# urgent-challenge/urgent2026_challenge_track1

Measured on AMD Instinct MI355X. Metric: utterances/sec (4 s @ 48 kHz) train step, higher is better.
Workload: dtype bf16

## Files before the change

include/urse.h:

```cpp
#ifndef URSE_H_
#define URSE_H_
#include <stdint.h>

#ifdef __cplusplus
extern "C" {
#endif

#define URSE_OK 0
#define URSE_ERR_INVALID_ARG (-1)
#define URSE_ERR_LAUNCH (-2)
#define URSE_ERR_UNSUPPORTED (-3)
#define URSE_ERR_RUNTIME (-4)

#define URSE_F32 0
#define URSE_BF16 1
#define URSE_F16 2
#define URSE_BF16_ACT_F16 3

#define URSE_WIN_RECT 0
#define URSE_WIN_HANN 1

int urse_version(void);
const char* urse_last_error(void);

#define URSE_KV_NT_BRES 0
#define URSE_KV_NT_RING 1
#define URSE_KV_NT_RING_WIDE 2
#define URSE_KV_NT_128 3
#define URSE_KV_NT_GROUPED_RING 4
#define URSE_KV_NT_GROUPED_128 5
#define URSE_KV_TN_RING 6
#define URSE_KV_TN_RING_T 7
#define URSE_KV_TN_DUAL 8
#define URSE_KV_TN_128 9
#define URSE_KV_TN_GROUPED 10
#define URSE_KV_LSTM_FWD_STREAM 11
#define URSE_KV_LSTM_FWD_WIDE 12
#define URSE_KV_LSTM_FWD_CLUSTER 13
#define URSE_KV_LSTM_FWD_CLUSTER2 14
#define URSE_KV_LSTM_BWD_STREAM16 15
#define URSE_KV_LSTM_BWD_STREAM32 16
#define URSE_KV_LSTM_BWD_CLUSTER 17
#define URSE_KV_LSTM_BWD_SPLIT 18
#define URSE_KV_STFT960 19
#define URSE_KV_STFT_GENERIC 20
#define URSE_KV_ISTFT_GENERIC 21
#define URSE_KV_ISTFT960 22
#define URSE_KV_LSTM_FWD_RW 23
#define URSE_KV_TN_ACT_F16 24
#define URSE_KV_LSTM_FWD_RWX 25
#define URSE_KV_LSTM_BWD_NSPLIT 26
#define URSE_KV_LSTM_FWD_CLUSTERX 27
#define URSE_KV_COUNT 32
int urse_launch_count(int variant);
int urse_launch_counts_reset(void);

int urse_stft_fwd(const float* wav, const int32_t* lens, float* spec, int B, int L, int n_fft, int hop,
                  int window, void* stream);
int urse_istft_fwd(const float* spec, float* wav, int B, int T, int n_fft, int hop, int L_out, int window,
                   void* stream);
int urse_istft_bwd(const float* grad_wav, float* grad_spec, int B, int T, int n_fft, int hop, int L_out,
                   int window, void* stream);

int urse_gemm_nt(const void* A, int64_t lda, const void* B, int64_t ldb, void* C, int64_t ldc, const float* bias,
                 const float* resid, int64_t ldr, int64_t M, int64_t N, int64_t K, int in_dtype, int out_dtype,
                 int act, void* stream);
int urse_gemm_nt_gnstats(const void* A, int64_t lda, const void* B, int64_t ldb, float* C, int64_t ldc, const float* bias,
                         const float* resid, int64_t ldr, int64_t M, int64_t N, int64_t K, int in_dtype, int act,
                         double* stats, int64_t rows_per_group, void* stream);
int urse_gemm_nt_gnbwd(const void* A, int64_t lda, const void* B, int64_t ldb, float* C, int64_t M, int64_t N, int64_t K, int in_dtype,
                       const float* x, const double* stats, const float* gamma, double* sums, float* dgamma, float* dbeta, float* part,
                       int slots, int64_t rows_per_group, float eps, void* stream);
int urse_gemm_nt_grouped(const void* descs, int groups, int max_blocks, int in_dtype, int out_dtype, int act,
                         void* stream);
int urse_gemm_nt_grouped_h(const void* descs, const int64_t* host_descs, int groups, int in_dtype, int out_dtype,
                           int act, void* stream);
int urse_gemm_tn(const void* A, int64_t lda, const void* B, int64_t ldb, float* C, int64_t ldc, float* colsum,
                 int64_t R, int64_t Mo, int64_t No, int64_t shift, int64_t inner, int64_t period,
                 int64_t invalid_step, int64_t perm_h, int dtype, int target_workgroups, void* stream);
int urse_gemm_tn_act_f16_supported(int64_t R, int64_t Mo, int64_t No, int64_t No2, int with_colsum, int64_t inner, int64_t period);
int urse_gemm_tn_dual(const void* A, int64_t lda, const void* B, int64_t ldb, float* C, int64_t ldc, float* colsum,
                      const void* B2, int64_t ldb2, float* C2, int64_t ldc2, int64_t R, int64_t Mo, int64_t No, int64_t No2,
                      int64_t shift, int64_t inner, int64_t period, int64_t invalid_step, int64_t perm_h, int dtype,
                      int target_workgroups, void* stream);
int urse_gemm_tn_grouped(const void* descs, int groups, int max_blocks, int dtype, void* stream);

int urse_groupnorm_fwd(const float* x, const float* gamma, const float* beta, const float* add, void* y, double* stats,
                       int B, int T, int Kg, int W, int N, int Np, int gstride, float eps, int out_dtype, void* y_bf16, void* stream);
int urse_groupnorm_stats(const float* x, double* stats, int B, int T, int Kg, int W, int N, void* stream);
int urse_groupnorm_apply(const float* x, const float* gamma, const float* beta, const float* add, void* y, const double* stats,
                         int B, int T, int Kg, int W, int N, int Np, int gstride, float eps, int out_dtype, void* y_bf16, void* stream);
int urse_groupnorm_bwd(const float* x, const float* dy, const double* stats, const float* gamma, const float* dres,
                       float* dx, float* dgamma, float* dbeta, double* sums, int B, int T, int Kg, int W, int N,
                       int gstride, float eps, void* dx_packed, int ldp, void* stream);
int urse_groupnorm_bwd_apply(const float* x, const float* dy, const double* stats, const double* sums, const float* gamma,
                             const float* dres, float* dx, int B, int T, int Kg, int W, int N, int gstride, float eps, void* dx_packed,
                             int ldp, void* stream);
int urse_pack2d(const void* in, int64_t ldi, int in_dtype, void* out, int64_t ldo, int out_dtype, int rows, int cols,
                int out_rows, int out_cols, int transpose, void* stream);

int urse_pack_segments(const float* in, void* out, const void* segs, int nseg, int blocks_per_seg, int transpose,
                       int out_dtype, void* stream);

int urse_lstm_pack(const float* wih, const float* whh, const float* bih, const float* bhh, void* wih_p, void* wihT_p,
                   float* bias, void* whh_frag, void* whhT_frag, int N, int Np, int H, int Hp, int dtype,
                   void* stream);

int urse_lstm_bidir_fwd(void* gx, int64_t ldg, const void* whh, void* hout, int64_t ldh, float* c, int H, int Hp,
                        int n_seq, int seq_len, int64_t inner, int64_t outer, int64_t stride, int save, int dtype,
                        int rows16, void* hout_bf16, void* stream);
int urse_lstm_pack_quads(const float* whh, void* out, int H, int Hp, int dtype, void* stream);
int urse_lstm_cluster_plan(int H, int Hp, int n_seq, int reserved_cus, int64_t* plan);
int urse_lstm_cluster_fwd(void* gx, int64_t ldg, const void* whhq, void* hout, int64_t ldh, float* c, void* hx,
                          void* counters, void* err_flag, int H, int Hp, int n_seq, int seq_len, int64_t inner,
                          int64_t outer, int64_t stride, int save, int reserved_cus, int xcd_aware, int dtype, void* hout_bf16,
                          void* stream);
int urse_lstm_clusterx_supported(int N, int Np, int H, int Hp);
int urse_lstm_clusterx_plan(int H, int Hp, int n_seq, int reserved_cus, int64_t* plan);
int urse_lstm_clusterx_hx_elems(int H, int Hp, int n_seq, int reserved_cus, int64_t* elems);
int urse_lstm_pack_quads_x(const float* wih, void* out, int N, int Np, int H, int dtype, void* stream);
int urse_lstm_clusterx_fwd(const void* xn, int64_t ldx, const void* wihq, const float* bias, const void* whhq, void* gates, int64_t ldg, void* hout,
                           int64_t ldh, float* c, void* hx, void* counters, void* err_flag, int N, int Np, int H, int Hp, int n_seq, int seq_len,
                           int64_t inner, int64_t outer, int64_t stride, int save, int reserved_cus, int xcd_aware, int dtype, void* hout_bf16,
                           void* stream);
int urse_lstm_cluster2_plan(int H, int Hp, int n_seq, int reserved_cus, int64_t* plan);
int urse_lstm_cluster2_fwd(void* gx, int64_t ldg, const void* whhq, void* hout, int64_t ldh, float* c, void* hx, void* err_flag,
                           int H, int Hp, int n_seq, int seq_len, int64_t inner, int64_t outer, int64_t stride, int save,
                           int reserved_cus, int dtype, void* stream);
int urse_lstm_pack_bwd_quads(const float* whh, void* out, int H, int C, void* stream);
int urse_lstm_cluster_bwd(const void* dh, int64_t ldd, void* gates, int64_t ldg, const float* c, const void* whhTq,
                          void* dgx, void* counters, void* err_flag, int H, int Hp, int n_seq, int seq_len, int64_t inner,
                          int64_t outer, int64_t stride, int reserved_cus, void* stream);
int urse_lstm_wide_supported(int H, int Hp);
int urse_lstm_pack_blocks(const float* whh, void* out, int H, int Hp, void* stream);
int urse_lstm_wide_fwd(void* gx, int64_t ldg, const void* whhb, void* hout, int64_t ldh, float* c, int H, int Hp,
// ... 146 lines not shown
```

urgent2026_challenge_track1_amd/csrc/gemm.hip:

```cpp
#include <stdlib.h>

#include <type_traits>
#include "urse_common.h"

namespace urse {

typedef __bf16 bf16x8_t __attribute__((ext_vector_type(8)));
typedef short short8_t __attribute__((ext_vector_type(8)));
typedef short short4_t __attribute__((ext_vector_type(4)));
typedef float f32x4_t __attribute__((ext_vector_type(4)));

struct GemmDesc {
  const char* A;
  const char* B;
  char* C;
  const float* bias;
  const float* resid;
  long lda, ldb, ldc;
  long M, N, K;
  long ldr;
};

constexpr int BM = 128, BN = 128;
constexpr int SLAB = 64;
// ... 1470 lines not shown
          }
        } else {
          const TO* sv = reinterpret_cast<const TO*>(src);
          for (int e = 0; e < EPC && col + e < d.N; ++e) {
            float f = to_f32<TO>(sv[e]);
            if (OS == 4 && d.resid && ACT != 2) f += d.resid[row * d.ldr + col + e];
            if (gst) {
              if (row < gbound) { gsa += f; gqa += f * f; } else { gsb += f; gqb += f * f; }
            }
            C[row * d.ldc + col + e] = from_f32<TO>(f);
            if constexpr (C2K) {
              if (C2) C2[row * d.ldr + col + e] = f32_to_bf16(f);
            }
          }
        }
      }
      ch += DCH;
      if (ch >= CPR) { ch -= CPR; ++lrow; }
    }
  }
  if constexpr (GNB) {
    __syncthreads();
    constexpr int SLOTS = NTHR / CPR;
    double* red = reinterpret_cast<double*>(lds);
    float4* pg = reinterpret_cast<float4*>(lds + 1024);
    float4* pb = pg + SLOTS * CPR;
    const double r0 = wave_sum_d((double)gsa), r1 = wave_sum_d((double)gqa), r2 = wave_sum_d((double)gsb), r3 = wave_sum_d((double)gqb);
    if (lane == 0) { red[w * 4] = r0; red[w * 4 + 1] = r1; red[w * 4 + 2] = r2; red[w * 4 + 3] = r3; }
    if (tid < SLOTS * CPR) {
      pg[tid] = make_float4(gnb_dg[0], gnb_dg[1], gnb_dg[2], gnb_dg[3]);
      pb[tid] = make_float4(gnb_db[0], gnb_db[1], gnb_db[2], gnb_db[3]);
    }
    __syncthreads();
    if (tid < 4) {
      double t = 0.0;
      for (int i = 0; i < NWV; ++i) t += red[i * 4 + tid];
      const long g = gnb_g0 + (tid >> 1);
      if ((tid < 2 || gnb_bound < m0 + BMX) && g * xt->rpg < d.M) atomicAdd(xt->gnb_sums + g * 2 + (tid & 1), t);
    }
    if (tid >= 64 && tid < 64 + CPR) {
      const int chf = tid - 64;
      const long col = n0 + chf * EPC;
      if (col < d.N) {
        float4 sg = make_float4(0.f, 0.f, 0.f, 0.f), sb = sg;
        for (int i = 0; i < SLOTS; ++i) {
          const float4 a = pg[i * CPR + chf], bq = pb[i * CPR + chf];
          sg.x += a.x; sg.y += a.y; sg.z += a.z; sg.w += a.w;
          sb.x += bq.x; sb.y += bq.y; sb.z += bq.z; sb.w += bq.w;
        }
        float* part = xt->gnb_part + (long)(blockIdx.x % xt->gnb_slots) * 2 * d.N;
        const float vg[4] = {sg.x, sg.y, sg.z, sg.w}, vb[4] = {sb.x, sb.y, sb.z, sb.w};
        for (int q = 0; q < 4 && col + q < d.N; ++q) {
          atomicAdd(part + col + q, vg[q]);
          atomicAdd(part + d.N + col + q, vb[q]);
        }
      }
    }
    return;
  }
  if (gst) {
    __syncthreads();
    double* red = reinterpret_cast<double*>(lds);
    const double r0 = wave_sum_d((double)gsa), r1 = wave_sum_d((double)gqa), r2 = wave_sum_d((double)gsb), r3 = wave_sum_d((double)gqb);
    if (lane == 0) { red[w * 4] = r0; red[w * 4 + 1] = r1; red[w * 4 + 2] = r2; red[w * 4 + 3] = r3; }
    __syncthreads();
    if (tid < 4) {
      double t = 0.0;
      for (int i = 0; i < NWV; ++i) t += red[i * 4 + tid];
      const long g = gidx + (tid >> 1);
      if (tid < 2 || gbound < m0 + BMX) {
        if (g * rpg < d.M) atomicAdd(gstats + g * 2 + (tid & 1), t);
      }
    }
  }
}

template <typename TO, int NTW, int ACT, int BMX, int WNC = 2, typename TI = bf16_t>
__global__ void __launch_bounds__(BMX / 64 * WNC * 64) gemm_nt_dma_kernel(GemmDesc d, NtExtra x) {
  gemm_nt_dma_body<TO, NTW, ACT, BMX, WNC, 0, TI>(d, x.gstats, x.rpg);
}

__global__ void __launch_bounds__(512) gemm_nt_dma_gnb_kernel(GemmDesc d, NtExtra x) {
  gemm_nt_dma_body<float, 7, 0, 256, 2, 1>(d, nullptr, 0, &x);
}

__global__ void gnb_fold_kernel(const float* __restrict__ part, int slots, int N, float* __restrict__ dgamma, float* __restrict__ dbeta) {
  const int c = blockIdx.x * blockDim.x + threadIdx.x;
  if (c >= N) return;
  float a = 0.f, b = 0.f;
  for (int s = 0; s < slots; ++s) { a += part[(long)s * 2 * N + c]; b += part[(long)s * 2 * N + N + c]; }
  dgamma[c] += a;
  dbeta[c] += b;
}

template <typename TO, int ACT, typename TI = bf16_t>
__global__ void __launch_bounds__(512) gemm_nt_dma_grouped_kernel(const GemmDesc* __restrict__ descs) {
  const GemmDesc d = descs[blockIdx.y];
  gemm_nt_dma_body<TO, 7, ACT, 256, 2, 0, TI>(d);
}

template <int ACT, typename TI = bf16_t>
__global__ void __launch_bounds__(512) gemm_nt_bres_kernel(GemmDesc d, int wg_per_slice) {
  constexpr int BMX = 256, NTW = 7, BNX = 224, NST = 3, STAGE = BMX * 64, KSTEPS = 7, BRES = KSTEPS * 14 * 1024;
  __shared__ __attribute__((aligned(1024))) char lds[BRES + NST * STAGE];
  char* ring = lds + BRES;
  const int tm = (int)((d.M + BMX - 1) / BMX);
  const int tile_n = blockIdx.x / wg_per_slice, part = blockIdx.x - tile_n * wg_per_slice;
  const long n0 = (long)tile_n * BNX;
  const int tid = threadIdx.x, lane = tid & 63;
  const int w = __builtin_amdgcn_readfirstlane(tid >> 6), wm = w >> 1, wn = w & 1;
  const int nk = (int)(d.K / 32);
  const char* zsrc = reinterpret_cast<const char*>(g_tn_zero_page) + lane * 16;
  const int srow = lane >> 2, schunk = (lane & 3) ^ ((lane >> 3) & 3);
  const int lc = lane & 15, lr = lane >> 4;
  const int foff = lc * 64 + ((lr ^ ((lc >> 1) & 3)) << 4);
  for (int blk = w; blk < nk * 14; blk += 8) {
    const int kt = blk / 14, b = blk - kt * 14;
    const long row = n0 + b * 16 + srow;
    glds16(row < d.N ? d.B + (row * d.ldb) * 2 + schunk * 16 + (long)kt * 64 : zsrc, lds + blk * 1024);
  }
  f32x4_t bv[NTW];
#pragma unroll
  for (int j = 0; j < NTW; ++j) {
    const long col = n0 + (wn * NTW + j) * 16 + lr * 4;
#pragma unroll
    for (int r = 0; r < 4; ++r) bv[j][r] = (d.bias && col + r < d.N) ? d.bias[col + r] : 0.f;
  }
  bf16_t* C = reinterpret_cast<bf16_t*>(d.C);
  auto tile_src = [&](int mt, const char* (&pa)[2], bool (&aok)[2]) __attribute__((always_inline)) {
#pragma unroll
    for (int j = 0; j < 2; ++j) {
      const long row = (long)mt * BMX + 16 * (2 * w + j) + srow;
      aok[j] = mt < tm && row < d.M;
      pa[j] = d.A + (row * d.lda) * 2 + schunk * 16;
    }
  };
  auto issue = [&](const char* (&pa)[2], bool (&aok)[2], int kt, int slot) __attribute__((always_inline)) {
#pragma unroll
    for (int j = 0; j < 2; ++j)
      glds16((kt < nk && aok[j]) ? pa[j] + (long)kt * 64 : zsrc, ring + slot * STAGE + (2 * w + j) * 1024);
  };
  const char* pa[2];
  bool aok[2];
  tile_src(part, pa, aok);
  issue(pa, aok, 0, 2);
  for (int mt = part; mt < tm; mt += wg_per_slice) {
    const long m0 = (long)mt * BMX;
    issue(pa, aok, 1, 0);
    f32x4_t acc[4][NTW];
#pragma unroll
    for (int i = 0; i < 4; ++i)
#pragma unroll
      for (int j = 0; j < NTW; ++j) acc[i][j] = f32x4_t{0.f, 0.f, 0.f, 0.f};
    int slot = 2;
    for (int kt = 0; kt < nk; ++kt) {
      asm volatile("s_waitcnt vmcnt(2)" ::: "memory");
      __builtin_amdgcn_s_barrier();
      int nslot = slot + 2;
      if (nslot >= NST) nslot -= NST;
      issue(pa, aok, kt + 2, nslot);
      const char* As = ring + slot * STAGE + wm * 4096 + foff;
      const char* Bs = lds + kt * (14 * 1024) + wn * NTW * 1024 + foff;
      short8_t a[4], b[NTW];
#pragma unroll
      for (int i = 0; i < 4; ++i) a[i] = *reinterpret_cast<const short8_t*>(As + i * 1024);
#pragma unroll
// ... 227 lines not shown
  else { set_error("gemm_nt: bad dtype %d/%d", in_dtype, out_dtype); return URSE_ERR_INVALID_ARG; }
  URSE_CHECK_LAUNCH("urse_gemm_nt");
  return URSE_OK;
}

static long g_nt_bres_min_n = getenv("URSE_NT_BRES_MIN_N") ? atol(getenv("URSE_NT_BRES_MIN_N")) : 448;
static int g_nt_bres_wgs = 256;
static int g_nt_wide_default = 1;
static long g_nt_wide_maxk = 256;

static int gemm_nt_impl(const void* A, int64_t lda, const void* B, int64_t ldb, void* C, int64_t ldc,
                        const float* bias, const float* resid, int64_t ldr, int64_t M, int64_t N, int64_t K,
                        int in_dtype, int out_dtype, int act, void* stream, double* gstats, long rpg, int* fused) {
  NtExtra xtra{};
  GemmDesc d;
  d.A = (const char*)A; d.B = (const char*)B; d.C = (char*)C; d.bias = bias; d.resid = resid;
  d.lda = lda; d.ldb = ldb; d.ldc = ldc; d.M = M; d.N = N; d.K = K; d.ldr = ldr;
  const bool in16 = in_dtype == URSE_BF16 || in_dtype == URSE_F16;
  const bool f16 = in_dtype == URSE_F16;
  URSE_CHECK_ARG(in16 || in_dtype == URSE_F32, "urse_gemm_nt: bad operand dtype %d", in_dtype);
  URSE_CHECK_ARG(out_dtype == URSE_F32 || (out_dtype == URSE_BF16 && !f16) || (out_dtype == URSE_F16 && f16),
                 "urse_gemm_nt: output dtype %d with operand dtype %d (16-bit outputs take the operands' format)", out_dtype, in_dtype);
  const bool out16 = out_dtype != URSE_F32;
  int rc = check_desc_host(d, in16 ? 2 : 4, "urse_gemm_nt");
  if (rc) return rc;
  URSE_CHECK_ARG(!resid || act == 2 || out_dtype == URSE_F32 || (in_dtype == URSE_F16 && out_dtype == URSE_F16 && act == 1),
                 "urse_gemm_nt: residual epilogue writes f32 (f16 operands with act 1: the aux slot is the bf16 copy of the output)");
  URSE_CHECK_ARG(act != 2 || resid, "urse_gemm_nt: act 2 (tanh backward) needs the aux operand");
  static const bool no_dma = getenv("URSE_NT_NO_DMA") != nullptr;
  const char* bres_env = getenv("URSE_NT_BRES");
  const int bres_mode = bres_env ? atoi(bres_env) : 1;
#ifdef URSE_EXPERIMENTS
  const long wreg_min_n = getenv("URSE_NT_WREG_MIN_N") ? atol(getenv("URSE_NT_WREG_MIN_N")) : 0;
  if (wreg_min_n > 0 && in_dtype == URSE_BF16 && out_dtype == URSE_BF16 && !no_dma && M >= 8192 && N >= wreg_min_n && K == 32 * WR_KS &&
      !resid && act != 2 && (ldc * 2) % 16 == 0 && ((uintptr_t)C % 16) == 0 && M * lda * 2 < 0xFFFFF000L && M * ldc * 2 < 0xFFFFF000L) {
    const int tn = (int)((N + WR_BNX - 1) / WR_BNX);
    int parts = 252 / tn;
    if (parts < 1) parts = 1;
    long rpp = (M + parts - 1) / parts;
    rpp = (rpp + WR_ROWS - 1) / WR_ROWS * WR_ROWS;
    dim3 grid((unsigned)(tn * parts));
    hipStream_t st = (hipStream_t)stream;
    note_launch(URSE_KV_NT_BRES);
    if (act == 0) hipLaunchKernelGGL(gemm_nt_wreg_kernel<0>, grid, dim3(448), 0, st, d, parts, rpp);
    else hipLaunchKernelGGL(gemm_nt_wreg_kernel<1>, grid, dim3(448), 0, st, d, parts, rpp);
    URSE_CHECK_LAUNCH("urse_gemm_nt");
    return URSE_OK;
  }
#endif
  if (bres_mode && in16 && out16 && !no_dma && M >= 8192 && N >= g_nt_bres_min_n && K % 32 == 0 &&
      K >= 96 && K <= 224 && !resid && act != 2 && (ldc * 2) % 16 == 0 && ((uintptr_t)C % 16) == 0) {
    const int tn = (int)((N + 223) / 224);
    int per = g_nt_bres_wgs / tn;
    if (per < 1) per = 1;
    dim3 grid((unsigned)(tn * per));
    hipStream_t st = (hipStream_t)stream;
    note_launch(URSE_KV_NT_BRES);
    if (f16) {
      if (act == 0) hipLaunchKernelGGL((gemm_nt_bres_kernel<0, f16_t>), grid, dim3(512), 0, st, d, per);
      else hipLaunchKernelGGL((gemm_nt_bres_kernel<1, f16_t>), grid, dim3(512), 0, st, d, per);
    } else if (act == 0) hipLaunchKernelGGL(gemm_nt_bres_kernel<0>, grid, dim3(512), 0, st, d, per);
    else hipLaunchKernelGGL(gemm_nt_bres_kernel<1>, grid, dim3(512), 0, st, d, per);
    URSE_CHECK_LAUNCH("urse_gemm_nt");
    return URSE_OK;
  }
  if (in16 && !no_dma && M >= 2048 && N >= 160 && K % 32 == 0 && K >= 96 && !(f16 && act == 2)) {
    const long pad7 = (N + 223) / 224 * 224, pad8 = (N + 255) / 256 * 256;
    int ntw = pad7 <= pad8 ? 7 : 8;
    if (const char* e = getenv("URSE_NT_NTW")) ntw = atoi(e) == 8 ? 8 : 7;
    int bmx = 256;
    if (const char* e = getenv("URSE_NT_BMX")) bmx = atoi(e) == 128 ? 128 : 256;
    int wide = g_nt_wide_default && K <= g_nt_wide_maxk && N >= 1792 && out_dtype == URSE_BF16 && (N + 447) / 448 * 448 <= pad7 + 64;
    if (const char* e = getenv("URSE_NT_WIDE")) wide = atoi(e) != 0 && N >= 448;
    if (f16) { wide = 0; bmx = 256; }
    const long tl = wide ? ((M + 127) / 128) * ((N + 447) / 448) : ((M + bmx - 1) / bmx) * ((N + 32L * ntw - 1) / (32L * ntw));
    URSE_CHECK_ARG(tl < (1L << 31), "urse_gemm_nt: too many tiles");
    dim3 grid((unsigned)tl);
    hipStream_t st = (hipStream_t)stream;
    if (gstats && out_dtype == URSE_F32 && act != 2 && !wide && rpg >= bmx) {
      xtra.gstats = gstats;
      xtra.rpg = rpg;
      if (fused) *fused = 1;
    }
#define URSE_NT_DMA(TO_, NTW_, ACT_, BMX_) \
  hipLaunchKernelGGL((gemm_nt_dma_kernel<TO_, NTW_, ACT_, BMX_>), grid, dim3(BMX_ * 2), 0, st, d, xtra)
#define URSE_NT_DMA_W(TO_, ACT_) \
  hipLaunchKernelGGL((gemm_nt_dma_kernel<TO_, 7, ACT_, 128, 4>), grid, dim3(512), 0, st, d, xtra)
#define URSE_NT_DMA_B(TO_, NTW_, ACT_) do { if (wide) URSE_NT_DMA_W(TO_, ACT_); else if (bmx == 128) URSE_NT_DMA(TO_, NTW_, ACT_, 128); else URSE_NT_DMA(TO_, NTW_, ACT_, 256); } while (0)
#define URSE_NT_DMA_ACT(TO_, NTW_) \
  do { if (act == 0) URSE_NT_DMA_B(TO_, NTW_, 0); else if (act == 1) URSE_NT_DMA_B(TO_, NTW_, 1); else URSE_NT_DMA_B(TO_, NTW_, 2); } while (0)
    note_launch(wide ? URSE_KV_NT_RING_WIDE : URSE_KV_NT_RING);
    if (f16) {
#define URSE_NT_DMA_H(TO_, NTW_, ACT_) hipLaunchKernelGGL((gemm_nt_dma_kernel<TO_, NTW_, ACT_, 256, 2, f16_t>), grid, dim3(512), 0, st, d, xtra)
#define URSE_NT_DMA_H_ACT(TO_, NTW_) do { if (act == 0) URSE_NT_DMA_H(TO_, NTW_, 0); else URSE_NT_DMA_H(TO_, NTW_, 1); } while (0)
      if (out_dtype == URSE_F16) { if (ntw == 7) URSE_NT_DMA_H_ACT(f16_t, 7); else URSE_NT_DMA_H_ACT(f16_t, 8); }
      else { if (ntw == 7) URSE_NT_DMA_H_ACT(float, 7); else URSE_NT_DMA_H_ACT(float, 8); }
    } else if (out_dtype == URSE_BF16) {
      if (ntw == 7) URSE_NT_DMA_ACT(bf16_t, 7); else URSE_NT_DMA_ACT(bf16_t, 8);
    } else {
      if (ntw == 7) URSE_NT_DMA_ACT(float, 7); else URSE_NT_DMA_ACT(float, 8);
    }
    URSE_CHECK_LAUNCH("urse_gemm_nt");
    return URSE_OK;
  }
  const long blocks = ((M + BM - 1) / BM) * ((N + BN - 1) / BN);
  URSE_CHECK_ARG(blocks < (1L << 31), "urse_gemm_nt: too many tiles");
  note_launch(URSE_KV_NT_128);
  return dispatch_nt(nullptr, d, 1, (int)blocks, in_dtype, out_dtype, act, (hipStream_t)stream);
}

extern "C" int urse_gemm_nt(const void* A, int64_t lda, const void* B, int64_t ldb, void* C, int64_t ldc,
                            const float* bias, const float* resid, int64_t ldr, int64_t M, int64_t N, int64_t K,
                            int in_dtype, int out_dtype, int act, void* stream) {
  return gemm_nt_impl(A, lda, B, ldb, C, ldc, bias, resid, ldr, M, N, K, in_dtype, out_dtype, act, stream, nullptr, 0, nullptr);
}

extern "C" int urse_gemm_nt_gnstats(const void* A, int64_t lda, const void* B, int64_t ldb, float* C, int64_t ldc,
                                    const float* bias, const float* resid, int64_t ldr, int64_t M, int64_t N, int64_t K,
                                    int in_dtype, int act, double* stats, int64_t rows_per_group, void* stream) {
  URSE_CHECK_ARG(stats && rows_per_group > 0 && M % rows_per_group == 0 && ldc == N && N % 4 == 0,
                 "urse_gemm_nt_gnstats: needs whole groups of rows, a dense output and N %% 4 == 0");
  const int groups = (int)(M / rows_per_group);
  (void)hipMemsetAsync(stats, 0, sizeof(double) * 2 * groups, (hipStream_t)stream);
  int fused = 0;
  int rc = gemm_nt_impl(A, lda, B, ldb, C, ldc, bias, resid, ldr, M, N, K, in_dtype, URSE_F32, act, stream, stats, rows_per_group,
                        &fused);
  if (rc || fused) return rc;
  return urse_groupnorm_stats(C, stats, groups, (int)rows_per_group, 1, (int)N, (int)N, stream);
}

extern "C" int urse_gemm_nt_gnbwd(const void* A, int64_t lda, const void* B, int64_t ldb, float* C, int64_t M, int64_t N, int64_t K,
                                  int in_dtype, const float* x, const double* stats, const float* gamma, double* sums, float* dgamma,
                                  float* dbeta, float* part, int slots, int64_t rows_per_group, float eps, void* stream) {
  URSE_CHECK_ARG(A && B && C && x && stats && gamma && sums && dgamma && dbeta && part && slots > 0 && rows_per_group > 0,
                 "urse_gemm_nt_gnbwd: bad argument");
  static const bool no_dma = getenv("URSE_NT_NO_DMA") != nullptr;
  if (no_dma || in_dtype != URSE_BF16 || M < 2048 || N < 160 || N > 224 || N % 4 || K % 32 || K < 96 || rows_per_group < 256 ||
      M % rows_per_group || ((uintptr_t)C % 16) || ((uintptr_t)x % 16)) {
    set_error("urse_gemm_nt_gnbwd: shape M%ld N%ld K%ld not served by the fused kernel", (long)M, (long)N, (long)K);
    return URSE_ERR_UNSUPPORTED;
  }
  GemmDesc d;
  d.A = (const char*)A; d.B = (const char*)B; d.C = (char*)C; d.bias = nullptr; d.resid = nullptr;
  d.lda = lda; d.ldb = ldb; d.ldc = N; d.M = M; d.N = N; d.K = K; d.ldr = 0;
  int rc = check_desc_host(d, 2, "urse_gemm_nt_gnbwd");
  if (rc) return rc;
  hipStream_t st = (hipStream_t)stream;
  const size_t sums_bytes = sizeof(double) * 2 * (size_t)(M / rows_per_group), part_bytes = sizeof(float) * 2 * (size_t)N * slots;
  if (reinterpret_cast<char*>(part) == reinterpret_cast<char*>(sums) + sums_bytes) {
    (void)hipMemsetAsync(sums, 0, sums_bytes + part_bytes, st);
  } else {
    (void)hipMemsetAsync(sums, 0, sums_bytes, st);
    (void)hipMemsetAsync(part, 0, part_bytes, st);
  }
  NtExtra xt{};
  xt.rpg = rows_per_group; xt.gnb_x = x; xt.gnb_stats = stats; xt.gnb_gamma = gamma; xt.gnb_sums = sums; xt.gnb_part = part;
  xt.gnb_slots = slots; xt.gnb_eps = eps;
  const long tl = (M + 255) / 256;
  URSE_CHECK_ARG(tl < (1L << 31), "urse_gemm_nt_gnbwd: too many tiles");
  note_launch(URSE_KV_NT_RING);
  hipLaunchKernelGGL(gemm_nt_dma_gnb_kernel, dim3((unsigned)tl), dim3(512), 0, st, d, xt);
  hipLaunchKernelGGL(gnb_fold_kernel, dim3((unsigned)((N + 255) / 256)), dim3(256), 0, st, part, slots, (int)N, dgamma, dbeta);
  URSE_CHECK_LAUNCH("urse_gemm_nt_gnbwd");
  return URSE_OK;
}

// ... 251 lines not shown
```

urgent2026_challenge_track1_amd/ops.py:

```python
import os

import torch

from . import _lib
from ._lib import call, require_cuda, stream_ptr

WIN_RECT, WIN_HANN = 0, 1
F32, BF16, F16 = 0, 1, 2
BF16_ACT_F16 = 3
HALF_TYPES = (torch.bfloat16, torch.float16)


def bwd_dtype(dtype):
    return torch.bfloat16 if dtype == torch.float16 else dtype

_timing = None


def enable_timing(names):
    global _timing
    _timing = {n: [] for n in names}


def disable_timing():
    global _timing
    t, _timing = _timing, None
    return t


def timed_call(tname, name, *args):
    if _timing is not None and tname in _timing:
        a, b = torch.cuda.Event(enable_timing=True), torch.cuda.Event(enable_timing=True)
        a.record()
        call(name, *args)
        b.record()
        _timing[tname].append((a, b))
    else:
        call(name, *args)


KERNEL_VARIANTS = ("nt_bres", "nt_ring", "nt_ring_wide", "nt_128", "nt_grouped_ring", "nt_grouped_128", "tn_ring", "tn_ring_t",
                   "tn_dual", "tn_128", "tn_grouped", "lstm_fwd_stream", "lstm_fwd_wide", "lstm_fwd_cluster",
                   "lstm_fwd_cluster2", "lstm_bwd_stream16", "lstm_bwd_stream32", "lstm_bwd_cluster", "lstm_bwd_split",
                   "stft960", "stft_generic", "istft_generic", "istft960", "lstm_fwd_rw", "tn_act_f16", "lstm_fwd_rwx", "lstm_bwd_nsplit",
                   "lstm_fwd_clusterx", "_unused28")


_PAGEABLE_UPLOADS = os.environ.get("URSE_PAGEABLE_UPLOADS", "0") == "1"


def upload(host_tensor, device, cached=False):
    if torch.device(device).type != "cuda":
        return host_tensor
    if _PAGEABLE_UPLOADS:
        return host_tensor.to(device)
    out = host_tensor.contiguous().pin_memory().to(device, non_blocking=True)
    if cached:
        ev = torch.cuda.Event()
        ev.record(torch.cuda.current_stream(device))
        ev.synchronize()
    return out


def launch_counts(reset=False):
    lib = _lib.load()
    out = {n: lib.urse_launch_count(i) for i, n in enumerate(KERNEL_VARIANTS)}
    if reset:
        lib.urse_launch_counts_reset()
    return out


def _f32c(t):
    return t.contiguous().float() if (t.dtype != torch.float32 or not t.is_contiguous()) else t


def stft_forward(wav, n_fft, hop, window=WIN_HANN, lens=None):
    require_cuda(wav)
    wav = _f32c(wav)
    B, L = wav.shape
    T, Fb = L // hop + 1, n_fft // 2 + 1
    spec = torch.empty(B, T, Fb, 2, device=wav.device, dtype=torch.float32)
    if lens is not None:
        if lens.device.type == "cpu":
            lens = upload(lens.to(torch.int32), wav.device)
        else:
            lens = lens.to(device=wav.device, dtype=torch.int32).contiguous()
    timed_call("stft_fwd", "stft_fwd", wav, lens, spec, B, L, n_fft, hop, window, stream_ptr())
    return torch.view_as_complex(spec)


class _ISTFT(torch.autograd.Function):
    @staticmethod
    def forward(ctx, spec_ri, n_fft, hop, length, window):
        B, T, Fb, _ = spec_ri.shape
        wav = torch.empty(B, length, device=spec_ri.device, dtype=torch.float32)
        call("istft_fwd", spec_ri, wav, B, T, n_fft, hop, length, window, stream_ptr())
        ctx.cfg = (B, T, Fb, n_fft, hop, length, window)
        return wav

    @staticmethod
    def backward(ctx, g):
        B, T, Fb, n_fft, hop, length, window = ctx.cfg
        g = _f32c(g)
        gs = torch.empty(B, T, Fb, 2, device=g.device, dtype=torch.float32)
        call("istft_bwd", g, gs, B, T, n_fft, hop, length, window, stream_ptr())
        return gs, None, None, None, None


def istft_forward(spec, n_fft, hop, length, window=WIN_HANN):
    if spec.is_complex():
        spec = torch.view_as_real(spec)
    require_cuda(spec)
    return _ISTFT.apply(_f32c(spec), n_fft, hop, int(length), window)


def _dt(t):
    if t.dtype == torch.bfloat16:
        return BF16
    if t.dtype == torch.float32:
        return F32
    if t.dtype == torch.float16:
        return F16
    raise TypeError("URSE GEMM operands are bf16, f16 or f32, got %s" % t.dtype)


def dtype_code(dtype):
    return {torch.float32: F32, torch.bfloat16: BF16, torch.float16: F16}[dtype]

# ... 882 lines not shown
```

Before: 256.1.

## Add persistent streaming NT GEMM kernel for narrow fp32 outputs with residual

Adds a persistent NT GEMM kernel that launches one workgroup per CU and loops over M tiles. The next tile's first K slabs are prefetched into the LDS ring while the current tile's epilogue runs, and the epilogue is staged through LDS so bias, residual and group-norm stats are applied in coalesced row sweeps with nontemporal stores. It is on by default for fp32-output, no-activation, N<=224 GEMMs that have a residual and enough tiles. The aim is to remove per-tile launch and drain overhead and to hide epilogue memory traffic, at the cost of extra barriers and fewer workgroups per CU.

```diff
diff --git a/include/urse.h b/include/urse.h
--- a/include/urse.h
+++ b/include/urse.h
@@ -51,6 +51,7 @@
 #define URSE_KV_LSTM_FWD_RWX 25
 #define URSE_KV_LSTM_BWD_NSPLIT 26
 #define URSE_KV_LSTM_FWD_CLUSTERX 27
+#define URSE_KV_NT_STREAM 28
 #define URSE_KV_COUNT 32
 int urse_launch_count(int variant);
 int urse_launch_counts_reset(void);
diff --git a/urgent2026_challenge_track1_amd/csrc/gemm.hip b/urgent2026_challenge_track1_amd/csrc/gemm.hip
--- a/urgent2026_challenge_track1_amd/csrc/gemm.hip
+++ b/urgent2026_challenge_track1_amd/csrc/gemm.hip
@@ -1576,6 +1576,187 @@
 
 __global__ void __launch_bounds__(512) gemm_nt_dma_gnb_kernel(GemmDesc d, NtExtra x) {
   gemm_nt_dma_body<float, 7, 0, 256, 2, 1>(d, nullptr, 0, &x);
+}
+
+template <int NTW, typename TI>
+__global__ void __launch_bounds__(512) gemm_nt_stream_kernel(GemmDesc d, NtExtra x) {
+  constexpr int BMX = 256, BNX = 32 * NTW, NWV = 8, NTHR = 512, NST = 4, STAGE = (BMX + 256) * 64, BOFF = BMX * 64;
+  constexpr int AI = 2, BI = 2;
+  constexpr int CP = BNX * 4 + 16, RPP = 32, STG = RPP * CP, CPR = BNX / 4;
+  constexpr int SW = (RPP * CPR + NTHR - 1) / NTHR;
+  static_assert(NST * STAGE + STG + BNX * 4 <= 160 * 1024, "ring + staging buffer + bias row exceed the LDS");
+  static_assert(BMX % (2 * RPP) == 0 && 2 * RPP == 64, "a wave's 64 rows are two passes");
+  __shared__ __attribute__((aligned(1024))) char lds[NST * STAGE + STG + BNX * 4];
+  char* const stg = lds + NST * STAGE;
+  const long tm = (d.M + BMX - 1) / BMX;
+  const long t0 = (long)blockIdx.x * tm / gridDim.x, t1 = ((long)blockIdx.x + 1) * tm / gridDim.x;
+  if (t0 >= t1) return;
+  const int tid = threadIdx.x, lane = tid & 63;
+  const int w = __builtin_amdgcn_readfirstlane(tid >> 6), wm = w >> 1, wn = w & 1;
+  const int nk = (int)(d.K / 32);
+  const char* zsrc = reinterpret_cast<const char*>(g_tn_zero_page) + lane * 16;
+  const int srow = lane >> 2, schunk = (lane & 3) ^ ((lane >> 3) & 3);
+  const int lc = lane & 15, lr = lane >> 4;
+  const int foff = lc * 64 + ((lr ^ ((lc >> 1) & 3)) << 4);
+
+  const char* pa[AI];
+  const char* pb[BI];
+  bool aok[AI], anx[AI], bok[BI], more = false;
+  const long tstride = (long)BMX * d.lda * 2;
+#pragma unroll
+  for (int j = 0; j < BI; ++j) {
+    const int rowl = 16 * (BI * w + j) + srow;
+    bok[j] = rowl < BNX && rowl < d.N;
+    pb[j] = d.B + ((long)rowl * d.ldb) * 2 + schunk * 16;
+  }
+  auto set_tile = [&](long t) {
+    more = t + 1 < t1;
+#pragma unroll
+    for (int j = 0; j < AI; ++j) {
+      const long row = t * BMX + 16 * (AI * w + j) + srow;
+      aok[j] = row < d.M;
+      anx[j] = more && row + BMX < d.M;
+      pa[j] = d.A + (row * d.lda) * 2 + schunk * 16;
+    }
+  };
+  auto issue = [&](int kt, int slot) {
+    char* sbase = lds + slot * STAGE;
+    const bool cur = kt < nk;
+    const long koff = (long)(cur ? kt : kt - nk) * 64;
+    const long aoff = cur ? koff : koff + tstride;
+#pragma unroll
+    for (int j = 0; j < AI; ++j) glds16((cur ? aok[j] : anx[j]) ? pa[j] + aoff : zsrc, sbase + (AI * w + j) * 1024);
+#pragma unroll
+    for (int j = 0; j < BI; ++j) glds16((bok[j] && (cur || more)) ? pb[j] + koff : zsrc, sbase + BOFF + (BI * w + j) * 1024);
+  };
+  set_tile(t0);
+#pragma unroll
+  for (int s = 0; s < NST - 1; ++s) issue(s, s);
+
+  float* const bls = reinterpret_cast<float*>(stg + STG);
+  if (tid < BNX) bls[tid] = (d.bias && tid < d.N) ? d.bias[tid] : 0.f;
+  static_assert(CPR <= 64 && SW * NWV == RPP, "one row per wave instruction");
+  const bool colok = lane * 4 < d.N;
+  const unsigned voff = colok ? lane * 16 : 0;
+  const bool has_res = d.resid != nullptr;
+  const bool gst = x.gstats != nullptr;
+  const long rpg = x.rpg;
+  float4 rr[SW];
+  auto rfetch = [&](long rowbase) {
+#pragma unroll
+    for (int it = 0; it < SW; ++it) {
+      const long row = rowbase + w + it * NWV;
+      const char* rb = (has_res && row < d.M) ? reinterpret_cast<const char*>(d.resid + row * d.ldr) : reinterpret_cast<const char*>(g_tn_zero_page);
+      rr[it] = *reinterpret_cast<const float4*>(rb + voff);
+    }
+  };
+
+  int slot = 0;
+#pragma unroll 1
+  for (long t = t0; t < t1; ++t) {
+    const long m0 = t * BMX;
+    if (t != t0) set_tile(t);
+    const long gidx = gst ? (long)((unsigned)m0 / (unsigned)rpg) : 0, gbound = gst ? (gidx + 1) * rpg : 0;
+    f32x4_t acc[4][NTW];
+#pragma unroll
+    for (int i = 0; i < 4; ++i)
+#pragma unroll
+      for (int j = 0; j < NTW; ++j) acc[i][j] = f32x4_t{0.f, 0.f, 0.f, 0.f};
+#pragma unroll 1
+    for (int kt = 0; kt < nk; ++kt) {
+      asm volatile("s_waitcnt vmcnt(8)" ::: "memory");
+      __builtin_amdgcn_s_barrier();
+      int nslot = slot + NST - 1;
+      if (nslot >= NST) nslot -= NST;
+      issue(kt + NST - 1, nslot);
+      const char* As = lds + slot * STAGE + wm * 4096 + foff;
+      const char* Bs = lds + slot * STAGE + BOFF + wn * NTW * 1024 + foff;
+      short8_t a[4];
+#pragma unroll
+      for (int i = 0; i < 4; ++i) a[i] = *reinterpret_cast<const short8_t*>(As + i * 1024);
+      short8_t b[NTW];
+#pragma unroll
+      for (int j = 0; j < NTW; ++j) b[j] = *reinterpret_cast<const short8_t*>(Bs + j * 1024);
+#pragma unroll
+      for (int j = 0; j < NTW; ++j)
+#pragma unroll
+        for (int i = 0; i < 4; ++i) acc[i][j] = Frag<TI>::mma(b[j], a[i], acc[i][j]);
+      if (++slot == NST) slot = 0;
+    }
+
+    float gsa = 0.f, gqa = 0.f, gsb = 0.f, gqb = 0.f;
+    auto stage = [&](auto I0) {
+      constexpr int i0 = decltype(I0)::value;
+      const int cb = (wn * NTW * 16 + lr * 4) * 4;
+      const char* bb = reinterpret_cast<const char*>(bls) + cb;
+      char* sb = stg + lc * CP + cb;
+#pragma unroll
+      for (int j = 0; j < NTW; ++j) {
+        const f32x4_t bj = *reinterpret_cast<const f32x4_t*>(bb + j * 64);
+#pragma unroll
+        for (int ii = 0; ii < 2; ++ii) {
+          const f32x4_t v = acc[i0 + ii][j] + bj;
+          *reinterpret_cast<f32x4_t*>(sb + ii * 16 * CP + j * 64) = v;
+        }
+      }
+    };
+    auto sweep = [&](long rowbase, bool more_passes) {
+      f32x4_t f[SW];
+#pragma unroll
+      for (int it = 0; it < SW; ++it) {
+        const int lrow = w + it * NWV;
+        const long row = rowbase + lrow;
+        f[it] = *reinterpret_cast<const f32x4_t*>(stg + lrow * CP + lane * 16);
+        const f32x4_t r = {rr[it].x, rr[it].y, rr[it].z, rr[it].w};
+        f[it] = has_res ? f[it] + r : f[it];
+        if (gst) {
+          const float sv = (f[it][0] + f[it][1]) + (f[it][2] + f[it][3]);
+          const float qv = (f[it][0] * f[it][0] + f[it][1] * f[it][1]) + (f[it][2] * f[it][2] + f[it][3] * f[it][3]);
+          const bool ok = colok && row < d.M, first = ok && row < gbound, second = ok && !first;
+          gsa += first ? sv : 0.f; gqa += first ? qv : 0.f;
+          gsb += second ? sv : 0.f; gqb += second ? qv : 0.f;
+        }
+      }
+      asm volatile("" : "+v"(gsa), "+v"(gqa), "+v"(gsb), "+v"(gqb));
+      if (more_passes) rfetch(rowbase + RPP);
+#pragma unroll
+      for (int it = 0; it < SW; ++it) {
+        const long row = rowbase + w + it * NWV;
+        if (row < d.M && colok) __builtin_nontemporal_store(f[it], reinterpret_cast<f32x4_t*>(d.C + row * d.ldc * 4 + voff));
+      }
+    };
+    auto lds_barrier = [&]() {
+      asm volatile("s_waitcnt lgkmcnt(0)" ::: "memory");
+      __builtin_amdgcn_s_barrier();
+    };
+    rfetch(m0);
+#pragma unroll
+    for (int q = 0; q < BMX / 64; ++q) {
+      const long r0 = m0 + q * 64;
+      lds_barrier();
+      if (wm == q) stage(std::integral_constant<int, 0>{});
+      lds_barrier();
+      sweep(r0, true);
+      lds_barrier();
+      if (wm == q) stage(std::integral_constant<int, 2>{});
+      lds_barrier();
+      sweep(r0 + RPP, q + 1 < BMX / 64);
+    }
+    if (gst) {
+      lds_barrier();
+      double* red = reinterpret_cast<double*>(stg);
+      const double s0 = wave_sum_d((double)gsa), s1 = wave_sum_d((double)gqa), s2 = wave_sum_d((double)gsb), s3 = wave_sum_d((double)gqb);
+      if (lane == 0) { red[w * 4] = s0; red[w * 4 + 1] = s1; red[w * 4 + 2] = s2; red[w * 4 + 3] = s3; }
+      lds_barrier();
+      if (tid < 4) {
+        double tot = 0.0;
+        for (int i = 0; i < NWV; ++i) tot += red[i * 4 + tid];
+        const long g = gidx + (tid >> 1);
+        if ((tid < 2 || gbound < m0 + BMX) && g * rpg < d.M) atomicAdd(x.gstats + g * 2 + (tid & 1), tot);
+      }
+    }
+  }
+  asm volatile("s_waitcnt vmcnt(0)" ::: "memory");
 }
 
 __global__ void gnb_fold_kernel(const float* __restrict__ part, int slots, int N, float* __restrict__ dgamma, float* __restrict__ dbeta) {
@@ -1969,6 +2150,22 @@
       xtra.rpg = rpg;
       if (fused) *fused = 1;
     }
+    const char* stream_env = getenv("URSE_NT_STREAM");
+    const int stream_mode = stream_env ? atoi(stream_env) : 1;
+    const bool stream_vec = M < (1L << 31) && N % 4 == 0 && ldc % 4 == 0 &&((uintptr_t)C % 16) == 0 && (!resid || (ldr % 4 == 0 && ((uintptr_t)resid % 16) == 0));
+    if (stream_mode && stream_vec && out_dtype == URSE_F32 && act == 0 && !wide && ntw == 7 && bmx == 256 && N <= 224) {
+      long wgs = device_cu_count();
+      if (const char* e = getenv("URSE_NT_STREAM_WGS")) { if (atol(e) > 0) wgs = atol(e); }
+      if (stream_mode == 2 || (resid && tl >= 2 * wgs)) {
+        const dim3 sgrid((unsigned)(tl < wgs ? tl : wgs));
+        note_launch(URSE_KV_NT_RING);
+        note_launch(URSE_KV_NT_STREAM);
+        if (f16) hipLaunchKernelGGL((gemm_nt_stream_kernel<7, f16_t>), sgrid, dim3(512), 0, st, d, xtra);
+        else hipLaunchKernelGGL((gemm_nt_stream_kernel<7, bf16_t>), sgrid, dim3(512), 0, st, d, xtra);
+        URSE_CHECK_LAUNCH("urse_gemm_nt");
+        return URSE_OK;
+      }
+    }
 #define URSE_NT_DMA(TO_, NTW_, ACT_, BMX_) \
   hipLaunchKernelGGL((gemm_nt_dma_kernel<TO_, NTW_, ACT_, BMX_>), grid, dim3(BMX_ * 2), 0, st, d, xtra)
 #define URSE_NT_DMA_W(TO_, ACT_) \
diff --git a/urgent2026_challenge_track1_amd/ops.py b/urgent2026_challenge_track1_amd/ops.py
--- a/urgent2026_challenge_track1_amd/ops.py
+++ b/urgent2026_challenge_track1_amd/ops.py
@@ -43,7 +43,7 @@
                    "tn_dual", "tn_128", "tn_grouped", "lstm_fwd_stream", "lstm_fwd_wide", "lstm_fwd_cluster",
                    "lstm_fwd_cluster2", "lstm_bwd_stream16", "lstm_bwd_stream32", "lstm_bwd_cluster", "lstm_bwd_split",
                    "stft960", "stft_generic", "istft_generic", "istft960", "lstm_fwd_rw", "tn_act_f16", "lstm_fwd_rwx", "lstm_bwd_nsplit",
-                   "lstm_fwd_clusterx", "_unused28")
+                   "lstm_fwd_clusterx", "nt_stream")
 
 
 _PAGEABLE_UPLOADS = os.environ.get("URSE_PAGEABLE_UPLOADS", "0") == "1"
```

Result: no change. 258.0, median of 6 (+0.8%).
